# DJT777/xlstm-yolo-clean

Measured on NVIDIA B200. Metric: mLSTM chunkwise fwd+bwd TFLOP/s (algorithmic, 14*L*d*(L+d) per chunk), higher is better.
Workload: dtype bf16

## Files before the change

xlstm_yolo_clean_b200/csrc/tensor_kernels.cu:

```cuda
#include <atomic>
#include <mutex>
#include <set>
#include <type_traits>
#include <utility>

#include "common.cuh"
#include "sm100.cuh"

namespace mlstm {
namespace {

using namespace sm100;

constexpr int LT = 128;
constexpr int kWorkers = 256;
constexpr int kTcThreads = 320;
constexpr int kCtlWarp = 8, kScanWarp = 9;
constexpr int kNbAB = kWorkers + 32;
constexpr int kNbC = kWorkers + 64;
constexpr float kLog2e = 1.4426950408889634f;
enum { NB_A = 1, NB_B = 2, NB_C = 3, NB_PAIR0 = 4 };

struct GateBuf {
  static constexpr int oB = 0, oI = LT, oPm = 2 * LT, oY = 3 * LT, oF = 4 * LT, oMt = 5 * LT, oNt = 6 * LT,
// ... 1050 lines not shown
              v[4 * j4 + 0] *= cf.x * r_t;
              v[4 * j4 + 1] *= cf.y * r_t;
              v[4 * j4 + 2] *= cf.z * r_t;
              v[4 * j4 + 3] *= cf.w * r_t;
              rs += (v[4 * j4 + 0] + v[4 * j4 + 1]) + (v[4 * j4 + 2] + v[4 * j4 + 3]);
            }
          } else if (u == rb) {
            tmem_ld32(tS + lane_base + u * 32, v);
#pragma unroll
            for (int j4 = 0; j4 < 8; ++j4) {
              const float4 y = *reinterpret_cast<const float4*>(sy + u * 32 + 4 * j4);
              const float yy[4] = {y.x, y.y, y.z, y.w};
#pragma unroll
              for (int e = 0; e < 4; ++e) {
                const int j = 4 * j4 + e;
                float pv = v[j] * ex2_approx(x_t + yy[e]);
                pv = (REV ? j >= lane : j <= lane) ? pv : 0.f;
                rs += pv;
                v[j] = pv;
              }
            }
          } else {
#pragma unroll
            for (int j = 0; j < 32; ++j) v[j] = 0.f;
          }
          store_row32<T>(sP, row, u * 32, v);
        }
        srs[ch * LT + row] = rs;
      }
      fence_proxy_async_smem();
      tc_fence_before_sync();
      named_arrive(NB_B, kNbAB);
      {
        const float ab = __expf(g - b_t + i_t - m_next);
#pragma unroll 1
        for (int hf = 0; hf < 2; ++hf) {
          float kb[32];
#pragma unroll
          for (int j = 0; j < 4; ++j) {
            uint4 u = *reinterpret_cast<const uint4*>(sK + ch * SM::kTile + swz128(row, hf * 32 + 8 * j));
            float2 a0 = unpack2<T>(u.x), a1 = unpack2<T>(u.y), a2 = unpack2<T>(u.z), a3 = unpack2<T>(u.w);
            kb[8 * j + 0] = a0.x * ab; kb[8 * j + 1] = a0.y * ab; kb[8 * j + 2] = a1.x * ab; kb[8 * j + 3] = a1.y * ab;
            kb[8 * j + 4] = a2.x * ab; kb[8 * j + 5] = a2.y * ab; kb[8 * j + 6] = a3.x * ab; kb[8 * j + 7] = a3.y * ab;
          }
          store_row32<T>(sKb, row, ch * 64 + hf * 32, kb);
          const float cs = warp_colsum32(kb, lane);
          snp[rb * D + ch * 64 + hf * 32 + lane] = cs;
        }
        fence_proxy_async_smem();
        named_arrive(NB_A, kNbAB);
      }
      mbar_wait(&bar_h, par, 7);
      tc_fence_after_sync();
      {
        const float bq = __expf(b_t + m_run - m_t) * p.scale;
        const float den = bq * (sqn[row] + sqn[LT + row]) + srs[row] + srs[LT + row];
        const float nmax = fmaxf(fabsf(den), __expf(-m_t));
        const float inv = 1.f / (nmax + p.eps);
#pragma unroll 1
        for (int hf = 0; hf < 2; ++hf) {
          uint32_t hi[32], hx[32];
          tmem_ld32_nowait(tHi + lane_base + ch * 64 + hf * 32, hi);
          tmem_ld32_nowait(tHx + lane_base + ch * 64 + hf * 32, hx);
          tmem_ld_wait();
          float o[32];
#pragma unroll
          for (int j = 0; j < 32; ++j) o[j] = (__uint_as_float(hi[j]) + bq * __uint_as_float(hx[j])) * inv;
          store_row32<T>(sH, row, ch * 64 + hf * 32, o);
        }
        if (ch == 0 && row < n_valid) {
          p.n_out[(int64_t)bh * p.S + t0 + row] = nmax;
          p.m_out[(int64_t)bh * p.S + t0 + row] = m_t;
        }
        if (EPI) {
          uint8_t* sub = sH + ch * SM::kTile;
          const int64_t tok = (int64_t)(t0 + row);
          if (p.h_plain && row < n_valid) {
            uint4* dst = reinterpret_cast<uint4*>((T*)p.h_plain + b * p.h_sb + hh * p.h_sh + tok * p.h_ss + ch * 64);
#pragma unroll
            for (int j = 0; j < 8; ++j) dst[j] = *reinterpret_cast<const uint4*>(sub + swz128(row, 8 * j));
          }
          const void* xrow = p.x ? (const void*)((const uint16_t*)p.x + b * p.x_sb + hh * p.x_sh + tok * p.x_ss + ch * 64) : nullptr;
          ln_epilogue_slice<T, 128, 64>(sub, [](int r, int cc) { return swz128(r, cc & 63); }, row, ch * 64, ch, NB_PAIR0 + rb,
                                        fsm + SM::fStat, fsm + SM::fPar, xrow, p.xy_f16 != 0, p.ln_eps, row < n_valid);
        }
      }
      mbar_wait(&bar_dc, par, 6);
      tc_fence_after_sync();
      {
#pragma unroll
        for (int hf = 0; hf < 2; ++hf) {
          float v[32], t32[32];
          tmem_ld32(tDC + lane_base + ch * 64 + hf * 32, v);
#pragma unroll
          for (int j = 0; j < 32; ++j) {
            Creg[hf * 32 + j] = gbar * Creg[hf * 32 + j] + v[j];
            t32[j] = Creg[hf * 32 + j];
          }
          store_row32<T>(sC, row, ch * 64 + hf * 32, t32);
        }
        if (tid < D) {
          sNn[tid] = gbar * sNc[tid] + ((snp[tid] + snp[D + tid]) + (snp[2 * D + tid] + snp[3 * D + tid]));
          mbar_arrive(&bar_n);
        }
      }
      fence_proxy_async_smem();
      tc_fence_before_sync();
      named_arrive(NB_C, kNbC);
      m_run = m_next;
      cur ^= 1;
    }
    if (p.c_last) {
      float* dst = p.c_last + ((int64_t)bh * D + row) * D + ch * 64;
#pragma unroll
      for (int j = 0; j < 64; ++j) dst[j] = Creg[j];
      if (tid < D) p.n_last[(int64_t)bh * D + tid] = fsm[SM::fN + cur * D + tid];
      if (tid == 0) p.m_last[bh] = m_run;
    }
  }
  tc_fence_before_sync();
  __syncthreads();
  if (warp == kCtlWarp) tmem_dealloc<512>(tmem);
}

struct TcBwParams {
  int B, NH, S, NT;
  float eps, scale;
  const void *ig, *fg;
  int64_t ig_sb, ig_sh, ig_ss, fg_sb, fg_sh, fg_ss;
  const float* m0;
  const float *n_out, *m_out, *dc_last;
  void *di, *df;
  int64_t di_sb, di_sh, di_ss, df_sb, df_sh, df_ss;
  float* dc0;
  int rev;
  int sig;
  float cap;
  int acc_qk, acc_v, acc_g;
  int cs_rows, cs_off;
#ifdef MLSTM_TC_PROFILE
  long long* prof;
#endif
};

template <int D_>
struct BwSmem {
  static constexpr int D = D_;
  static constexpr int kTile = Lay<D>::kTile;
  static constexpr int kPTile = LT * 128;
  static constexpr int kState = Lay<D>::kState;
  static constexpr int kNST = D == 64 ? 1 : 2;
  static constexpr int kStage = 4 * kTile + kState;
  static constexpr int oQ = 0, oK = kTile, oV = 2 * kTile, odH = 3 * kTile, oCs = 4 * kTile;
  static constexpr int oQt = kNST * kStage;
  static constexpr int oSb = oQt + kTile;
  static constexpr int odS = oSb + 2 * kPTile;
  static constexpr int odQ = odS + 2 * kPTile;
  static constexpr int odV = odQ + kTile;
  static constexpr int odK = odV + kTile;
  static constexpr int odC = odK + kTile;
  static constexpr int oSmall = odC + kState;
  static constexpr int fGates = 0, fPart = 2 * GateBuf::kFloats, kSmallFloats = fPart + 12 * LT;
  static constexpr int kBytes = oSmall + kSmallFloats * 4 + 1024;
  static constexpr uint32_t kLoadBytes = 4 * kTile + kState;
  static constexpr bool kAlias = D == 64;
  static constexpr uint32_t cS = 0, cdSb = 128;
  static constexpr uint32_t cdV1 = D == 64 ? 0 : 256, cdV2 = cdV1 + D, cdK1 = D == 64 ? 128 : 320, cdK2 = cdK1 + D,
                            cdQa = D == 64 ? 256 : 384, cdQb = cdQa + D, cddC = D == 64 ? 384 : 448;
};

template <typename T, int D, bool REV, typename TO>
__global__ void __launch_bounds__(kTcThreads, 1)
tc_bw(const __grid_constant__ CUtensorMap mapQ, const __grid_constant__ CUtensorMap mapK,
          const __grid_constant__ CUtensorMap mapV, const __grid_constant__ CUtensorMap mapdH,
          const __grid_constant__ CUtensorMap mapCs, const __grid_constant__ CUtensorMap mapdQ,
          const __grid_constant__ CUtensorMap mapdK, const __grid_constant__ CUtensorMap mapdV, TcBwParams p) {
  constexpr bool kBf16 = std::is_same<T, __nv_bfloat16>::value;
  using SM = BwSmem<D>;
  using L = Lay<D>;
  constexpr int CW = L::CW;
  TC_PROF(200, 0);
  TC_PROF_CTA(0);
  extern __shared__ uint8_t smem_raw[];
  uint8_t* smem = smem_raw + ((1024u - (smem_u32(smem_raw) & 1023u)) & 1023u);
  uint8_t* sQ = smem + SM::oQ;
  uint8_t* sK = smem + SM::oK;
  uint8_t* sV = smem + SM::oV;
  uint8_t* sdH = smem + SM::odH;
  uint8_t* sQt = smem + SM::oQt;
  uint8_t* sSb = smem + SM::oSb;
  uint8_t* sdS = smem + SM::odS;
  uint8_t* sdQ = smem + SM::odQ;
  uint8_t* sdV = smem + SM::odV;
  uint8_t* sdK = smem + SM::odK;
  uint8_t* sCs = smem + SM::oCs;
  uint8_t* sdC = smem + SM::odC;
  float* fsm = (float*)(smem + SM::oSmall);
  __shared__ uint64_t bar_full[SM::kNST], bar_s, bar_q, bar_v, bar_k, bar_d, bar_b, bar_st, bar_g[2];
  __shared__ uint32_t tmem_base_s;

  const int tid = threadIdx.x, lane = tid & 31;
  const int warp = __shfl_sync(0xffffffffu, tid >> 5, 0);
  const int bh = blockIdx.x, b = bh / p.NH, hh = bh % p.NH;

  auto mt = [&](int c) { return REV ? p.NT - 1 - c : c; };
  auto load_stage = [&](int s, int c) {
    uint8_t* base = smem + s * SM::kStage;
    mbar_expect_tx(&bar_full[s], SM::kLoadBytes);
    tma_load_4d(base + SM::oQ, &mapQ, &bar_full[s], 0, mt(c) * LT, hh, b);
    tma_load_4d(base + SM::oK, &mapK, &bar_full[s], 0, mt(c) * LT, hh, b);
    tma_load_4d(base + SM::oV, &mapV, &bar_full[s], 0, mt(c) * LT, hh, b);
    tma_load_4d(base + SM::odH, &mapdH, &bar_full[s], 0, mt(c) * LT, hh, b);
    tma_load_4d(base + SM::oCs, &mapCs, &bar_full[s], 0, mt(c) * p.cs_rows + p.cs_off, hh, b);
  };
  if (tid == kCtlWarp * 32) {
    for (int s = 0; s < SM::kNST; ++s) mbar_init(&bar_full[s], 1);
    fence_mbar_init();
    grid_dep_wait();
    for (int s = 0; s < SM::kNST && s < p.NT; ++s) load_stage(s, p.NT - 1 - s);
  }
  if (tid == 0) {
    mbar_init(&bar_s, 1);
    mbar_init(&bar_b, 1);
    mbar_init(&bar_st, 1);
    mbar_init(&bar_q, 1);
    mbar_init(&bar_v, 1);
    mbar_init(&bar_k, 1);
    mbar_init(&bar_d, 1);
    mbar_init(&bar_g[0], 1);
    mbar_init(&bar_g[1], 1);
    fence_mbar_init();
  }
  if (warp == kCtlWarp) {
    tmem_alloc<512>(&tmem_base_s);
    if (lane == 0) {
      prefetch_tmap(&mapQ); prefetch_tmap(&mapK); prefetch_tmap(&mapV); prefetch_tmap(&mapdH);
      prefetch_tmap(&mapCs); prefetch_tmap(&mapdQ); prefetch_tmap(&mapdK); prefetch_tmap(&mapdV);
    }
  }
  grid_dep_wait();
  grid_dep_launch();
  const int rb = warp & 3, ch = (warp >> 2) & 1;
  const int row = rb * 32 + lane;
  const uint32_t lane_base = (uint32_t)(rb * 32) << 16;
  const int drow = rb * 16 + (lane & 15);
  const bool owns_c = warp < kCtlWarp && lane < 16 && rb * 16 < D;
  float dCreg[CW];
#pragma unroll
  for (int j = 0; j < CW; ++j) dCreg[j] = 0.f;
  if (warp < kCtlWarp) {
    if (p.dc_last && owns_c) {
      const float* src = p.dc_last + ((int64_t)bh * D + drow) * D + ch * CW;
#pragma unroll
      for (int j = 0; j < CW; ++j) dCreg[j] = src[j];
    }
    if (owns_c) store_cols<T, D>(sdC, drow, ch * CW, dCreg);
    fence_proxy_async_smem();
  }
  tc_fence_before_sync();
  __syncthreads();
  tc_fence_after_sync();
  const uint32_t tmem = tmem_base_s;
  const uint32_t tS = tmem + SM::cS, tdSb = tmem + SM::cdSb;
  const uint32_t tdV1 = tmem + SM::cdV1, tdV2 = tmem + SM::cdV2, tdK1 = tmem + SM::cdK1, tdK2 = tmem + SM::cdK2;
  const uint32_t tdQa = tmem + SM::cdQa, tdQb = tmem + SM::cdQb, tddC = tmem + SM::cddC;

  const T* ip = (const T*)p.ig + b * p.ig_sb + hh * p.ig_sh;
  const T* fp = (const T*)p.fg + b * p.fg_sb + hh * p.fg_sh;
  const float* mo = p.m_out + (int64_t)bh * p.S;
  const float* no = p.n_out + (int64_t)bh * p.S;
  if (warp == kCtlWarp) {
    constexpr uint32_t id_s = umma_idesc(128, 128, false, false, kBf16);
    constexpr uint32_t id_c = umma_idesc(64, D, true, true, kBf16);
    constexpr uint32_t id_k_mn = umma_idesc(128, D, false, true, kBf16);
    constexpr uint32_t id_mn_mn = umma_idesc(128, D, true, true, kBf16);
    constexpr uint32_t id_k_k = umma_idesc(128, D, false, false, kBf16);
    const uint64_t kQ0 = L::desc(smem_u32(sQ), 0), mQ0 = L::desc(smem_u32(sQ), SM::kTile);
    const uint64_t kK0 = L::desc(smem_u32(sK), 0), mK0 = L::desc(smem_u32(sK), SM::kTile);
    const uint64_t kV0 = L::desc(smem_u32(sV), 0);
    const uint64_t kH0 = L::desc(smem_u32(sdH), 0), mH0 = L::desc(smem_u32(sdH), SM::kTile);
    const uint64_t kCs0 = L::desc(smem_u32(sCs), 0);
    const uint64_t mQt = L::desc(smem_u32(sQt), D == 64 ? SM::kTile : 0);
    const uint64_t mSb = umma_smem_desc(smem_u32(sSb), SM::kPTile, 1024);
    const uint64_t kdS = umma_smem_desc(smem_u32(sdS), 0, 1024), mdS = umma_smem_desc(smem_u32(sdS), SM::kPTile, 1024);
    const uint64_t kdC = L::desc(smem_u32(sdC), 0), mdC = L::desc(smem_u32(sdC), SM::kState);
    auto issue_s = [&](int it) {
      const int s = it % SM::kNST;
      const uint32_t so = (uint32_t)s * SM::kStage;
      const uint64_t kQ = umma_desc_advance(kQ0, so), kK = umma_desc_advance(kK0, so);
      const uint64_t kH = umma_desc_advance(kH0, so), kV = umma_desc_advance(kV0, so);
      mbar_wait(&bar_full[s], (it / SM::kNST) & 1, 11);
      tc_fence_after_sync();
#pragma unroll
      for (int kk = 0; kk < D / 16; ++kk)
        umma_f16(tS, umma_desc_advance(kQ, kk * 32), umma_desc_advance(kK, kk * 32), id_s, kk > 0);
#pragma unroll
      for (int kk = 0; kk < D / 16; ++kk)
        umma_f16(tdSb, umma_desc_advance(kH, kk * 32), umma_desc_advance(kV, kk * 32), id_s, kk > 0);
      umma_commit(&bar_s);
    };

    if (elect_one()) issue_s(0);
    __syncwarp();

    for (int it = 0; it < p.NT; ++it) {
      const int c = p.NT - 1 - it, pb = it & 1;
      const uint32_t par = it & 1;
      const int t0 = mt(c) * LT, n_valid = min(LT, p.S - t0);
      const uint32_t so = (uint32_t)(it % SM::kNST) * SM::kStage;
      const uint64_t kQ = umma_desc_advance(kQ0, so), mQ = umma_desc_advance(mQ0, so);
      const uint64_t kK = umma_desc_advance(kK0, so), mK = umma_desc_advance(mK0, so);
      const uint64_t kV = umma_desc_advance(kV0, so), kCs = umma_desc_advance(kCs0, so);
      const uint64_t kH = umma_desc_advance(kH0, so), mH = umma_desc_advance(mH0, so);
      TC_PROF(it, 9);
      if (SM::kNST == 1 && c > 0 && lane == 0) {
        const int r = mt(c - 1) * LT;
        tma_prefetch_4d(&mapQ, 0, r, hh, b);
        tma_prefetch_4d(&mapK, 0, r, hh, b);
        tma_prefetch_4d(&mapV, 0, r, hh, b);
        tma_prefetch_4d(&mapdH, 0, r, hh, b);
        tma_prefetch_4d(&mapCs, 0, mt(c - 1) * p.cs_rows + p.cs_off, hh, b);
      }
      named_sync(NB_B, kNbAB);
      TC_PROF(it, 10);
      if (elect_one()) {
        tc_fence_after_sync();
#pragma unroll
        for (int kk = 0; kk < LT / 16; ++kk)
          umma_f16(tdK1, umma_desc_advance(mdS, kk * 2048), umma_desc_advance(mQ, kk * L::kAdvMN), id_mn_mn, kk > 0);
#pragma unroll
        for (int kk = 0; kk < D / 16; ++kk)
          umma_f16(tdK2, umma_desc_advance(kV, kk * 32), umma_desc_advance(kdC, kk * 32), id_k_k, kk > 0);
        umma_commit(&bar_k);
#pragma unroll
        for (int kk = 0; kk < LT / 16; ++kk)
          umma_f16(tdQa, umma_desc_advance(kdS, (kk / 4) * SM::kPTile + (kk % 4) * 32), umma_desc_advance(mK, kk * L::kAdvMN),
                   id_k_mn, kk > 0);
#pragma unroll
        for (int kk = 0; kk < D / 16; ++kk)
          umma_f16(tdQb, umma_desc_advance(kH, kk * 32), umma_desc_advance(kCs, kk * 32), id_k_k, kk > 0);
        umma_commit(&bar_q);
#pragma unroll
        for (int kk = 0; kk < D / 16; ++kk)
          umma_f16(tdV2, umma_desc_advance(kK, kk * 32), umma_desc_advance(mdC, kk * L::kAdvMN), id_k_mn, kk > 0);
        umma_commit(&bar_b);
      }
      __syncwarp();
      if (lane == 0) {
        tma_store_wait_read<0>();
        mbar_arrive(&bar_st);
      }
      __syncwarp();
      TC_PROF(it, 11);
      named_sync(NB_A, kNbAB);
      TC_PROF(it, 12);
      if (elect_one()) {
#pragma unroll
        for (int kk = 0; kk < LT / 16; ++kk)
          umma_f16(tddC, umma_desc_advance(mQt, kk * L::kAdvMN), umma_desc_advance(mH, kk * L::kAdvMN), id_c, kk > 0);
        umma_commit(&bar_d);
#pragma unroll
        for (int kk = 0; kk < LT / 16; ++kk)
          umma_f16(tdV1, umma_desc_advance(mSb, kk * 2048), umma_desc_advance(mH, kk * L::kAdvMN), id_mn_mn, kk > 0);
        umma_commit(&bar_v);
        if (!SM::kAlias && c > 0) issue_s(it + 1);
        if (SM::kNST == 1) {
          if (c > 0) {
            const int r = mt(c - 1) * LT;
            mbar_expect_tx(&bar_full[0], SM::kLoadBytes);
            mbar_wait(&bar_k, par, 21);
            tma_load_4d(sQ, &mapQ, &bar_full[0], 0, r, hh, b);
            tma_load_4d(sV, &mapV, &bar_full[0], 0, r, hh, b);
            mbar_wait(&bar_q, par, 24);
            tma_load_4d(sCs, &mapCs, &bar_full[0], 0, mt(c - 1) * p.cs_rows + p.cs_off, hh, b);
            mbar_wait(&bar_b, par, 22);
            tma_load_4d(sK, &mapK, &bar_full[0], 0, r, hh, b);
            mbar_wait(&bar_v, par, 25);
            tma_load_4d(sdH, &mapdH, &bar_full[0], 0, r, hh, b);
          }
        } else if (c >= SM::kNST) {
          mbar_wait(&bar_v, par, 25);
          load_stage(it % SM::kNST, c - SM::kNST);
        }
      }
      __syncwarp();
      TC_PROF(it, 13);
      named_sync(NB_C, kNbC);
      TC_PROF(it, 14);
      if (lane == 0) {
        if (p.acc_qk) {
          tma_reduce_add_4d(&mapdQ, sdQ, 0, t0, hh, b);
          tma_reduce_add_4d(&mapdK, sdK, 0, t0, hh, b);
        } else {
          tma_store_4d(&mapdQ, sdQ, 0, t0, hh, b);
          tma_store_4d(&mapdK, sdK, 0, t0, hh, b);
        }
        if (p.acc_v) tma_reduce_add_4d(&mapdV, sdV, 0, t0, hh, b);
        else tma_store_4d(&mapdV, sdV, 0, t0, hh, b);
        tma_store_commit();
      }
      __syncwarp();
      if (SM::kAlias && c > 0 && elect_one()) issue_s(it + 1);
      __syncwarp();
    }
    if (lane == 0) tma_store_wait_all<0>();
  } else if (warp == kScanWarp) {
    struct TileRaw {
      GateRaw<T> g;
      float4 mt, nt;
      float m_prev, m_next;
    };
    auto raw_of = [&](int c) {
      TileRaw r;
      const int t0 = mt(c) * LT, n_valid = min(LT, p.S - t0);
      r.g = load_gate_raw<T>(ip + (int64_t)t0 * p.ig_ss, p.ig_ss, fp + (int64_t)t0 * p.fg_ss, p.fg_ss, n_valid);
      if (lane * 4 < n_valid) {
        r.mt = *reinterpret_cast<const float4*>(mo + t0 + lane * 4);
        r.nt = *reinterpret_cast<const float4*>(no + t0 + lane * 4);
      } else {
        r.mt = make_float4(0.f, 0.f, 0.f, 0.f);
        r.nt = make_float4(1.f, 1.f, 1.f, 1.f);
      }
      if (!REV) {
        r.m_prev = c > 0 ? mo[t0 - 1] : (p.m0 ? p.m0[bh] : 0.f);
        r.m_next = mo[t0 + n_valid - 1];
      } else {
        r.m_prev = c > 0 ? mo[t0 + LT] : (p.m0 ? p.m0[bh] : 0.f);
        r.m_next = mo[t0];
      }
      return r;
    };
    auto publish = [&](float* gb, const TileRaw& r) {
      gate_scan_regs(gb, r.g, REV, p.sig != 0, p.cap);
      reinterpret_cast<float4*>(gb + GateBuf::oMt)[lane] = r.mt;
      reinterpret_cast<float4*>(gb + GateBuf::oNt)[lane] = r.nt;
      if (lane == 0) {
        gb[GateBuf::oScal + 2] = r.m_prev;
        gb[GateBuf::oScal + 3] = r.m_next;
      }
    };

    TileRaw raw = raw_of(p.NT - 1);
    float carry = 0.f;
    for (int n = 0; n < p.NT + 2; ++n) {
      if (n >= 2) {
      const int it = n - 2;
      const int c = p.NT - 1 - it, pb = it & 1;
      const int t0 = mt(c) * LT, n_valid = min(LT, p.S - t0);
      named_sync(NB_C, kNbC);
      {
        const float* sp = fsm + SM::fPart + pb * 6 * LT;
        const float* gb = fsm + SM::fGates + pb * GateBuf::kFloats;
        float acc[4], di[4];
#pragma unroll
        for (int e = 0; e < 4; ++e) {
          const int t = lane * 4 + e;
          acc[e] = (sp[0 * LT + t] + sp[1 * LT + t]) - (sp[2 * LT + t] + sp[3 * LT + t]);
          di[e] = sp[4 * LT + t] + sp[5 * LT + t];
        }
        float incl, own;
        if (!REV) {
          acc[2] += acc[3];
          acc[1] += acc[2];
          acc[0] += acc[1];
          incl = own = acc[0];
#pragma unroll
          for (int o = 1; o < 32; o <<= 1) {
            float u = __shfl_down_sync(0xffffffffu, incl, o);
            if (lane + o < 32) incl += u;
          }
        } else {
          acc[1] += acc[0];
          acc[2] += acc[1];
          acc[3] += acc[2];
          incl = own = acc[3];
#pragma unroll
          for (int o = 1; o < 32; o <<= 1) {
            float u = __shfl_up_sync(0xffffffffu, incl, o);
            if (lane >= o) incl += u;
          }
        }
        const float excl = incl - own + carry;
        TO* dip = (TO*)p.di + b * p.di_sb + hh * p.di_sh;
        TO* dfp = (TO*)p.df + b * p.df_sb + hh * p.df_sh;
#pragma unroll
        for (int e = 0; e < 4; ++e) {
          const int t = lane * 4 + e;
          if (t < n_valid) {
            const float dsig = p.sig ? 1.f - __expf(gb[GateBuf::oI + t]) : 1.f;
            float gi = di[e] * dsig * gb[GateBuf::oDi + t];
            float gf = (acc[e] + excl) * sigmoid_neg_f32(gb[GateBuf::oF + t]) * gb[GateBuf::oDf + t];
            TO* pi = dip + (int64_t)(t0 + t) * p.di_ss;
            TO* pf = dfp + (int64_t)(t0 + t) * p.df_ss;
            if (p.acc_g) {
              gi += to_f32<TO>(*pi);
              gf += to_f32<TO>(*pf);
            }
            *pi = from_f32<TO>(gi);
            *pf = from_f32<TO>(gf);
          }
        }
        carry += __shfl_sync(0xffffffffu, incl, REV ? 31 : 0);
      }
      __syncwarp();
      }
      if (n < p.NT) {
        publish(fsm + SM::fGates + (n & 1) * GateBuf::kFloats, raw);
        __syncwarp();
        if (lane == 0) mbar_arrive(&bar_g[n & 1]);
        if (n + 1 < p.NT) raw = raw_of(p.NT - 2 - n);
      }
    }
  } else {
    for (int it = 0; it < p.NT; ++it) {
      const int pb = it & 1;
      const uint32_t par = it & 1;
      const float* gb = fsm + SM::fGates + pb * GateBuf::kFloats;
      float* spart = fsm + SM::fPart + pb * 6 * LT;
      const int n_valid = min(LT, p.S - mt(p.NT - 1 - it) * LT);
      const bool valid = row < n_valid;
      const uint32_t so = (uint32_t)(it % SM::kNST) * SM::kStage;

      TC_PROF(it, 0);
      mbar_wait(&bar_g[pb], (it >> 1) & 1, 12);
      const float g = gb[GateBuf::oScal], m_prev = gb[GateBuf::oScal + 2], m_next = gb[GateBuf::oScal + 3];
      const float b_t = gb[GateBuf::oB + row], i_t = gb[GateBuf::oI + row];
      const float m_t = gb[GateBuf::oMt + row], n_t = gb[GateBuf::oNt + row];
      const float rinv = valid ? 1.f / (n_t + p.eps) : 0.f;
      const float bbar = valid ? __expf(b_t + m_prev - m_t) : 0.f;
      const float abar = __expf(g - b_t + i_t - m_next);
      const float gbar = __expf(g + m_prev - m_next);
      TC_PROF(it, 1);
      mbar_wait(&bar_full[it % SM::kNST], (it / SM::kNST) & 1, 13);
      uint32_t qs[CW / 2];
      {
        const float wq = p.scale * bbar * rinv;
#pragma unroll
        for (int j = 0; j < CW / 8; ++j) {
          const uint32_t off = L::swz(row, ch * CW + 8 * j);
          uint4 u = *reinterpret_cast<const uint4*>(sQ + so + off);
          qs[4 * j] = u.x; qs[4 * j + 1] = u.y; qs[4 * j + 2] = u.z; qs[4 * j + 3] = u.w;
          float2 a0 = unpack2<T>(u.x), a1 = unpack2<T>(u.y), a2 = unpack2<T>(u.z), a3 = unpack2<T>(u.w);
          u.x = pack2<T>(a0.x * wq, a0.y * wq);
          u.y = pack2<T>(a1.x * wq, a1.y * wq);
          u.z = pack2<T>(a2.x * wq, a2.y * wq);
          u.w = pack2<T>(a3.x * wq, a3.y * wq);
          *reinterpret_cast<uint4*>(sQt + off) = u;
        }
      }
      mbar_wait(&bar_s, par, 14);
      tc_fence_after_sync();
      TC_PROF(it, 2);
      {
        const float x_t = valid ? (b_t - m_t) * kLog2e + log2f(rinv) : -INFINITY;
        const float* sy = gb + GateBuf::oY;
        const float* scf = gb + GateBuf::oCf;
#pragma unroll 1
        for (int u = ch; u < 4; u += 2) {
          float v[32], w[32];
          if (REV ? u >= rb : u <= rb) {
            uint32_t rv[32], rw[32];
            tmem_ld32_nowait(tS + lane_base + u * 32, rv);
            tmem_ld32_nowait(tdSb + lane_base + u * 32, rw);
            tmem_ld_wait();
            if (u != rb) {
              const float r_t = ex2_approx(x_t + gb[GateBuf::oScal + 4 + u]);
#pragma unroll
              for (int j4 = 0; j4 < 8; ++j4) {
                const float4 cf = *reinterpret_cast<const float4*>(scf + u * 32 + 4 * j4);
                const float cc[4] = {cf.x, cf.y, cf.z, cf.w};
#pragma unroll
                for (int e = 0; e < 4; ++e) {
                  const int j = 4 * j4 + e;
                  const float wg = cc[e] * r_t;
                  v[j] = __uint_as_float(rv[j]) * wg;
                  w[j] = __uint_as_float(rw[j]) * wg;
                }
              }
            } else {
#pragma unroll
              for (int j4 = 0; j4 < 8; ++j4) {
                const float4 y = *reinterpret_cast<const float4*>(sy + u * 32 + 4 * j4);
                const float yy[4] = {y.x, y.y, y.z, y.w};
#pragma unroll
                for (int e = 0; e < 4; ++e) {
                  const int j = 4 * j4 + e;
                  float wg = ex2_approx(x_t + yy[e]);
                  wg = (REV ? j >= lane : j <= lane) ? wg : 0.f;
                  v[j] = __uint_as_float(rv[j]) * wg;
                  w[j] = __uint_as_float(rw[j]) * wg;
                }
              }
            }
          } else {
            if (it > 0) continue;
#pragma unroll
            for (int j = 0; j < 32; ++j) { v[j] = 0.f; w[j] = 0.f; }
          }
          store_row32<T>(sSb, row, u * 32, v);
          store_row32<T>(sdS, row, u * 32, w);
        }
      }
      fence_proxy_async_smem();
      tc_fence_before_sync();
      named_arrive(NB_B, kNbAB);
      TC_PROF(it, 3);
      uint32_t ks[CW / 2], vs[CW / 2];
#pragma unroll
      for (int j = 0; j < CW / 8; ++j) {
        const uint32_t off = L::swz(row, ch * CW + 8 * j);
        uint4 uk = *reinterpret_cast<const uint4*>(sK + so + off);
        ks[4 * j] = uk.x; ks[4 * j + 1] = uk.y; ks[4 * j + 2] = uk.z; ks[4 * j + 3] = uk.w;
        uint4 uv = *reinterpret_cast<const uint4*>(sV + so + off);
        vs[4 * j] = uv.x; vs[4 * j + 1] = uv.y; vs[4 * j + 2] = uv.z; vs[4 * j + 3] = uv.w;
      }
      fence_proxy_async_smem();
      named_arrive(NB_A, kNbAB);
      TC_PROF(it, 4);
      {
        uint32_t ra[CW], rq[CW];
        float o[CW];
        float dot;
        mbar_wait(&bar_k, par, 18);
        tc_fence_after_sync();
        TC_PROF(it, 5);
        tmem_ld_nowait(tdK1 + lane_base + ch * CW, ra);
        tmem_ld_nowait(tdK2 + lane_base + ch * CW, rq);
        tmem_ld_wait();
        dot = 0.f;
#pragma unroll
        for (int j = 0; j < CW / 2; ++j) {
          o[2 * j] = p.scale * __uint_as_float(ra[2 * j]) + abar * __uint_as_float(rq[2 * j]);
          o[2 * j + 1] = p.scale * __uint_as_float(ra[2 * j + 1]) + abar * __uint_as_float(rq[2 * j + 1]);
          float2 kv = unpack2<T>(ks[j]);
          dot += kv.x * o[2 * j] + kv.y * o[2 * j + 1];
        }
        mbar_wait(&bar_st, par, 19);
        store_cols<TO, D>(sdK, row, ch * CW, o);
        spart[(1 * 2 + ch) * LT + row] = dot;
        mbar_wait(&bar_q, par, 16);
        tc_fence_after_sync();
        TC_PROF(it, 6);
        tmem_ld_nowait(tdQa + lane_base + ch * CW, ra);
        tmem_ld_nowait(tdQb + lane_base + ch * CW, rq);
        tmem_ld_wait();
        const float wb = bbar * rinv;
        dot = 0.f;
#pragma unroll
        for (int j = 0; j < CW / 2; ++j) {
          o[2 * j] = p.scale * (__uint_as_float(ra[2 * j]) + wb * __uint_as_float(rq[2 * j]));
          o[2 * j + 1] = p.scale * (__uint_as_float(ra[2 * j + 1]) + wb * __uint_as_float(rq[2 * j + 1]));
          float2 qv = unpack2<T>(qs[j]);
          dot += qv.x * o[2 * j] + qv.y * o[2 * j + 1];
        }
        store_cols<TO, D>(sdQ, row, ch * CW, o);
        spart[(0 * 2 + ch) * LT + row] = dot;
      }
      mbar_wait(&bar_d, par, 15);
      tc_fence_after_sync();
      TC_PROF(it, 7);
      {
        float v[CW];
        tmem_ld(tddC + lane_base + ch * CW, v);
        if (owns_c) {
#pragma unroll
          for (int j = 0; j < CW; ++j) dCreg[j] = gbar * dCreg[j] + v[j];
          store_cols<T, D>(sdC, drow, ch * CW, dCreg);
        }
      }
      {
        uint32_t ra[CW], rq[CW];
        float o[CW];
        float dot;
        mbar_wait(&bar_v, par, 17);
        tc_fence_after_sync();
        tmem_ld_nowait(tdV1 + lane_base + ch * CW, ra);
        tmem_ld_nowait(tdV2 + lane_base + ch * CW, rq);
        tmem_ld_wait();
        dot = 0.f;
#pragma unroll
        for (int j = 0; j < CW / 2; ++j) {
          o[2 * j] = p.scale * __uint_as_float(ra[2 * j]) + abar * __uint_as_float(rq[2 * j]);
          o[2 * j + 1] = p.scale * __uint_as_float(ra[2 * j + 1]) + abar * __uint_as_float(rq[2 * j + 1]);
          float2 vv = unpack2<T>(vs[j]);
          dot += vv.x * o[2 * j] + vv.y * o[2 * j + 1];
        }
        store_cols<TO, D>(sdV, row, ch * CW, o);
        spart[(2 * 2 + ch) * LT + row] = dot;
      }
      fence_proxy_async_smem();
      tc_fence_before_sync();
      named_arrive(NB_C, kNbC);
      TC_PROF(it, 8);
    }
    if (p.dc0 && owns_c) {
      float* dst = p.dc0 + ((int64_t)bh * D + drow) * D + ch * CW;
#pragma unroll
      for (int j = 0; j < CW; ++j) dst[j] = dCreg[j];
    }
  }
  TC_PROF(200, 1);
  tc_fence_before_sync();
  __syncthreads();
  TC_PROF(200, 2);
  TC_PROF_CTA(1);
  if (warp == kCtlWarp) tmem_dealloc<512>(tmem);
}

#ifdef MLSTM_TC_PROFILE
std::atomic<long long*> g_prof{nullptr};
#define TC_SET_PROF(p, off) (p).prof = g_prof.load() ? g_prof.load() + (off) : nullptr
#else
#define TC_SET_PROF(p, off)
#endif

int num_sms() {
  static int n = 0;
  if (!n) {
    int dev = 0;
    cudaGetDevice(&dev);
    cudaDeviceGetAttribute(&n, cudaDevAttrMultiProcessorCount, dev);
  }
  return n;
}

template <typename K>
cudaError_t ensure_smem(K kern, int bytes) {
  static std::mutex mu;
  static std::set<std::pair<const void*, int>> done;
  int dev = 0;
  cudaGetDevice(&dev);
  const std::pair<const void*, int> key(reinterpret_cast<const void*>(kern), dev);
  {
    std::lock_guard<std::mutex> g(mu);
    if (done.count(key)) return cudaSuccess;
  }
  cudaError_t e = cudaFuncSetAttribute(kern, cudaFuncAttributeMaxDynamicSharedMemorySize, bytes);
  if (e == cudaSuccess) {
    std::lock_guard<std::mutex> g(mu);
    done.insert(key);
  }
  return e;
}

int pdl_mode() {
  static int v = -1;
  if (v < 0) {
    const char* e = getenv("MLSTM_B200_PDL");
    v = e ? (e[0] - '0') : 2;
    if (v < 0 || v > 2) v = 2;
  }
  return v;
}
template <typename... KArgs, typename... Args>
cudaError_t launch_pdl(bool use_pdl, void (*kern)(KArgs...), int grid, int block, size_t smem, cudaStream_t st, Args&&... args) {
  cudaLaunchConfig_t cfg = {};
  cfg.gridDim = dim3(grid), cfg.blockDim = dim3(block), cfg.dynamicSmemBytes = smem, cfg.stream = st;
  cudaLaunchAttribute attr[1];
  attr[0].id = cudaLaunchAttributeProgrammaticStreamSerialization;
  attr[0].val.programmaticStreamSerializationAllowed = 1;
  cfg.attrs = attr, cfg.numAttrs = use_pdl ? 1 : 0;
  return cudaLaunchKernelEx(&cfg, kern, std::forward<Args>(args)...);
}

template <typename T, int D>
int launch_fw(const TcFwParams& p, const CUtensorMap& mq, const CUtensorMap& mk, const CUtensorMap& mv,
              const CUtensorMap& mh, const CUtensorMap& mcs, cudaStream_t st) {
  using SM = FwSmem<D>;
  auto kern = p.epi ? (p.rev ? tc_fw<T, D, true, true> : tc_fw<T, D, false, true>)
                    : (p.rev ? tc_fw<T, D, true, false> : tc_fw<T, D, false, false>);
  MLSTM_CUDA_CHECK(ensure_smem(kern, SM::kBytes));
  MLSTM_CUDA_CHECK(launch_pdl(pdl_mode() != 0, kern, p.B * p.NH, kTcThreads, SM::kBytes, st, mq, mk, mv, mh, mcs, p));
  count_launch();
  MLSTM_CUDA_CHECK(cudaGetLastError());
  return 0;
}

template <typename... KArgs, typename... Args>
cudaError_t launch_pair_pdl(bool use_pdl, void (*kern)(KArgs...), int grid, int block, size_t smem, cudaStream_t st,
                            Args&&... args) {
  cudaLaunchConfig_t cfg = {};
  cfg.gridDim = dim3(grid), cfg.blockDim = dim3(block), cfg.dynamicSmemBytes = smem, cfg.stream = st;
  cudaLaunchAttribute attr[2];
  attr[0].id = cudaLaunchAttributeClusterDimension;
  attr[0].val.clusterDim.x = 2, attr[0].val.clusterDim.y = 1, attr[0].val.clusterDim.z = 1;
  attr[1].id = cudaLaunchAttributeProgrammaticStreamSerialization;
  attr[1].val.programmaticStreamSerializationAllowed = 1;
  cfg.attrs = attr, cfg.numAttrs = use_pdl ? 2 : 1;
  return cudaLaunchKernelEx(&cfg, kern, std::forward<Args>(args)...);
}

template <typename T, int D>
auto fw_rect_kernel(bool epi, bool rev) {
  return epi ? (rev ? tc_fw_rect<T, D, true, true> : tc_fw_rect<T, D, false, true>)
             : (rev ? tc_fw_rect<T, D, true, false> : tc_fw_rect<T, D, false, false>);
}

template <typename T, int D>
int launch_fw_rect(const TcFwParams& p, const CUtensorMap& mq, const CUtensorMap& mk, const CUtensorMap& mv,
                   const CUtensorMap& mh, const CUtensorMap& mcs, cudaStream_t st) {
  using SM = FwSmem<D>;
  auto kern = fw_rect_kernel<T, D>(p.epi != 0, p.rev != 0);
  if (p.epi) {
    MLSTM_CUDA_CHECK(ensure_smem(kern, SM::kBytesPair));
    MLSTM_CUDA_CHECK(launch_pair_pdl(pdl_mode() != 0, kern, 2 * p.B * p.NH, kTcThreads, SM::kBytesPair, st, mq, mk, mv, mh, mcs, p));
  } else {
    MLSTM_CUDA_CHECK(ensure_smem(kern, SM::kBytes));
    MLSTM_CUDA_CHECK(launch_pdl(pdl_mode() != 0, kern, 2 * p.B * p.NH, kTcThreads, SM::kBytes, st, mq, mk, mv, mh, mcs, p));
  }
  count_launch();
  MLSTM_CUDA_CHECK(cudaGetLastError());
  return 0;
}

template <typename T>
int launch_fw_d128(const TcFwParams& p, const CUtensorMap& mq, const CUtensorMap& mk, const CUtensorMap& mv,
                   const CUtensorMap& mh, const CUtensorMap& mcs, cudaStream_t st) {
  auto kern = p.epi ? (p.rev ? tc_fw_d128<T, true, true> : tc_fw_d128<T, false, true>)
                    : (p.rev ? tc_fw_d128<T, true, false> : tc_fw_d128<T, false, false>);
  MLSTM_CUDA_CHECK(ensure_smem(kern, FwSmem128::kBytes));
  kern<<<p.B * p.NH, kTcThreads, FwSmem128::kBytes, st>>>(mq, mk, mv, mh, mcs, p);
  count_launch();
  MLSTM_CUDA_CHECK(cudaGetLastError());
  return 0;
}

template <typename T, int D, typename TO = T>
int launch_bw(const TcBwParams& p, const CUtensorMap& mq, const CUtensorMap& mk, const CUtensorMap& mv,
              const CUtensorMap& mdh, const CUtensorMap& mcs, const CUtensorMap& mdq, const CUtensorMap& mdk,
              const CUtensorMap& mdv, cudaStream_t st) {
  using SM = BwSmem<D>;
  auto kern = p.rev ? tc_bw<T, D, true, TO> : tc_bw<T, D, false, TO>;
  MLSTM_CUDA_CHECK(ensure_smem(kern, SM::kBytes));
  MLSTM_CUDA_CHECK(launch_pdl(pdl_mode() == 1, kern, p.B * p.NH, kTcThreads, SM::kBytes, st, mq, mk, mv, mdh, mcs, mdq, mdk, mdv, p));
  MLSTM_CUDA_CHECK(cudaGetLastError());
  return 0;
}

bool tma_ok(const mlstm_b200_tensor& t) {
  return ((uintptr_t)t.ptr & 15) == 0 && t.stride[3] == 1 && (t.stride[0] % 8) == 0 && (t.stride[1] % 8) == 0 &&
         (t.stride[2] % 8) == 0;
}
// ... 366 lines not shown
```

Before: 251.1.

## Fold gate scales into operands and accumulate dK/dQ partials in single TMEM tiles

The backward tensor-core kernel now pre-scales dH (instead of Q) and V by their gate factors in shared memory. This lets the two dK matmuls and the two dQ matmuls accumulate into one TMEM region each, instead of two regions combined later in registers. The dC state-gradient GEMM is issued in the first batch, the Cs state tile gets its own barrier so most MMAs can start before it arrives, and the MMA/TMA issue order and barrier set are reorganized. The aim is to remove epilogue FMAs and TMEM loads and to overlap the loads better. In exchange there are extra shared-memory rewrites of V, possible bf16 rounding of the pre-scaled operands, and more intricate synchronization.

```diff
diff --git a/xlstm_yolo_clean_b200/csrc/tensor_kernels.cu b/xlstm_yolo_clean_b200/csrc/tensor_kernels.cu
--- a/xlstm_yolo_clean_b200/csrc/tensor_kernels.cu
+++ b/xlstm_yolo_clean_b200/csrc/tensor_kernels.cu
@@ -1226,8 +1226,8 @@
   static constexpr int kNST = D == 64 ? 1 : 2;
   static constexpr int kStage = 4 * kTile + kState;
   static constexpr int oQ = 0, oK = kTile, oV = 2 * kTile, odH = 3 * kTile, oCs = 4 * kTile;
-  static constexpr int oQt = kNST * kStage;
-  static constexpr int oSb = oQt + kTile;
+  static constexpr int odHt = kNST * kStage;
+  static constexpr int oSb = odHt + kTile;
   static constexpr int odS = oSb + 2 * kPTile;
   static constexpr int odQ = odS + 2 * kPTile;
   static constexpr int odV = odQ + kTile;
@@ -1236,11 +1236,10 @@
   static constexpr int oSmall = odC + kState;
   static constexpr int fGates = 0, fPart = 2 * GateBuf::kFloats, kSmallFloats = fPart + 12 * LT;
   static constexpr int kBytes = oSmall + kSmallFloats * 4 + 1024;
-  static constexpr uint32_t kLoadBytes = 4 * kTile + kState;
-  static constexpr bool kAlias = D == 64;
-  static constexpr uint32_t cS = 0, cdSb = 128;
-  static constexpr uint32_t cdV1 = D == 64 ? 0 : 256, cdV2 = cdV1 + D, cdK1 = D == 64 ? 128 : 320, cdK2 = cdK1 + D,
-                            cdQa = D == 64 ? 256 : 384, cdQb = cdQa + D, cddC = D == 64 ? 384 : 448;
+  static constexpr uint32_t kLoadBytes = 4 * kTile;
+  static constexpr uint32_t cS = 0, cdSb = 128, cddC = cdSb;
+  static constexpr uint32_t cdQ = 256, cdK = cdQ + D, cdV1 = cdK + D, cdV2 = cdV1 + D;
+  static_assert(cdV2 + D <= 512, "TMEM columns");
 };
 
 template <typename T, int D, bool REV, typename TO>
@@ -1261,7 +1260,7 @@
   uint8_t* sK = smem + SM::oK;
   uint8_t* sV = smem + SM::oV;
   uint8_t* sdH = smem + SM::odH;
-  uint8_t* sQt = smem + SM::oQt;
+  uint8_t* sdHt = smem + SM::odHt;
   uint8_t* sSb = smem + SM::oSb;
   uint8_t* sdS = smem + SM::odS;
   uint8_t* sdQ = smem + SM::odQ;
@@ -1270,7 +1269,7 @@
   uint8_t* sCs = smem + SM::oCs;
   uint8_t* sdC = smem + SM::odC;
   float* fsm = (float*)(smem + SM::oSmall);
-  __shared__ uint64_t bar_full[SM::kNST], bar_s, bar_q, bar_v, bar_k, bar_d, bar_b, bar_st, bar_g[2];
+  __shared__ uint64_t bar_full[SM::kNST], bar_cs[SM::kNST], bar_s, bar_q, bar_v, bar_k, bar_st, bar_g[2];
   __shared__ uint32_t tmem_base_s;
 
   const int tid = threadIdx.x, lane = tid & 31;
@@ -1285,22 +1284,24 @@
     tma_load_4d(base + SM::oK, &mapK, &bar_full[s], 0, mt(c) * LT, hh, b);
     tma_load_4d(base + SM::oV, &mapV, &bar_full[s], 0, mt(c) * LT, hh, b);
     tma_load_4d(base + SM::odH, &mapdH, &bar_full[s], 0, mt(c) * LT, hh, b);
-    tma_load_4d(base + SM::oCs, &mapCs, &bar_full[s], 0, mt(c) * p.cs_rows + p.cs_off, hh, b);
+    mbar_expect_tx(&bar_cs[s], SM::kState);
+    tma_load_4d(base + SM::oCs, &mapCs, &bar_cs[s], 0, mt(c) * p.cs_rows + p.cs_off, hh, b);
   };
   if (tid == kCtlWarp * 32) {
-    for (int s = 0; s < SM::kNST; ++s) mbar_init(&bar_full[s], 1);
+    for (int s = 0; s < SM::kNST; ++s) {
+      mbar_init(&bar_full[s], 1);
+      mbar_init(&bar_cs[s], 1);
+    }
     fence_mbar_init();
     grid_dep_wait();
     for (int s = 0; s < SM::kNST && s < p.NT; ++s) load_stage(s, p.NT - 1 - s);
   }
   if (tid == 0) {
     mbar_init(&bar_s, 1);
-    mbar_init(&bar_b, 1);
     mbar_init(&bar_st, 1);
     mbar_init(&bar_q, 1);
     mbar_init(&bar_v, 1);
     mbar_init(&bar_k, 1);
-    mbar_init(&bar_d, 1);
     mbar_init(&bar_g[0], 1);
     mbar_init(&bar_g[1], 1);
     fence_mbar_init();
@@ -1336,8 +1337,8 @@
   tc_fence_after_sync();
   const uint32_t tmem = tmem_base_s;
   const uint32_t tS = tmem + SM::cS, tdSb = tmem + SM::cdSb;
-  const uint32_t tdV1 = tmem + SM::cdV1, tdV2 = tmem + SM::cdV2, tdK1 = tmem + SM::cdK1, tdK2 = tmem + SM::cdK2;
-  const uint32_t tdQa = tmem + SM::cdQa, tdQb = tmem + SM::cdQb, tddC = tmem + SM::cddC;
+  const uint32_t tdQ = tmem + SM::cdQ, tdK = tmem + SM::cdK, tdV1 = tmem + SM::cdV1, tdV2 = tmem + SM::cdV2;
+  const uint32_t tddC = tmem + SM::cddC;
 
   const T* ip = (const T*)p.ig + b * p.ig_sb + hh * p.ig_sh;
   const T* fp = (const T*)p.fg + b * p.fg_sb + hh * p.fg_sh;
@@ -1349,12 +1350,12 @@
     constexpr uint32_t id_k_mn = umma_idesc(128, D, false, true, kBf16);
     constexpr uint32_t id_mn_mn = umma_idesc(128, D, true, true, kBf16);
     constexpr uint32_t id_k_k = umma_idesc(128, D, false, false, kBf16);
-    const uint64_t kQ0 = L::desc(smem_u32(sQ), 0), mQ0 = L::desc(smem_u32(sQ), SM::kTile);
+    const uint64_t kQ0 = L::desc(smem_u32(sQ), 0), mQ0 = L::desc(smem_u32(sQ), D == 64 ? SM::kTile : 0);
     const uint64_t kK0 = L::desc(smem_u32(sK), 0), mK0 = L::desc(smem_u32(sK), SM::kTile);
     const uint64_t kV0 = L::desc(smem_u32(sV), 0);
     const uint64_t kH0 = L::desc(smem_u32(sdH), 0), mH0 = L::desc(smem_u32(sdH), SM::kTile);
     const uint64_t kCs0 = L::desc(smem_u32(sCs), 0);
-    const uint64_t mQt = L::desc(smem_u32(sQt), D == 64 ? SM::kTile : 0);
+    const uint64_t kHt = L::desc(smem_u32(sdHt), 0), mHt = L::desc(smem_u32(sdHt), SM::kTile);
     const uint64_t mSb = umma_smem_desc(smem_u32(sSb), SM::kPTile, 1024);
     const uint64_t kdS = umma_smem_desc(smem_u32(sdS), 0, 1024), mdS = umma_smem_desc(smem_u32(sdS), SM::kPTile, 1024);
     const uint64_t kdC = L::desc(smem_u32(sdC), 0), mdC = L::desc(smem_u32(sdC), SM::kState);
@@ -1385,7 +1386,7 @@
       const uint64_t kQ = umma_desc_advance(kQ0, so), mQ = umma_desc_advance(mQ0, so);
       const uint64_t kK = umma_desc_advance(kK0, so), mK = umma_desc_advance(mK0, so);
       const uint64_t kV = umma_desc_advance(kV0, so), kCs = umma_desc_advance(kCs0, so);
-      const uint64_t kH = umma_desc_advance(kH0, so), mH = umma_desc_advance(mH0, so);
+      const uint64_t mH = umma_desc_advance(mH0, so);
       TC_PROF(it, 9);
       if (SM::kNST == 1 && c > 0 && lane == 0) {
         const int r = mt(c - 1) * LT;
@@ -1401,23 +1402,31 @@
         tc_fence_after_sync();
 #pragma unroll
         for (int kk = 0; kk < LT / 16; ++kk)
-          umma_f16(tdK1, umma_desc_advance(mdS, kk * 2048), umma_desc_advance(mQ, kk * L::kAdvMN), id_mn_mn, kk > 0);
-#pragma unroll
-        for (int kk = 0; kk < D / 16; ++kk)
-          umma_f16(tdK2, umma_desc_advance(kV, kk * 32), umma_desc_advance(kdC, kk * 32), id_k_k, kk > 0);
-        umma_commit(&bar_k);
-#pragma unroll
-        for (int kk = 0; kk < LT / 16; ++kk)
-          umma_f16(tdQa, umma_desc_advance(kdS, (kk / 4) * SM::kPTile + (kk % 4) * 32), umma_desc_advance(mK, kk * L::kAdvMN),
-                   id_k_mn, kk > 0);
-#pragma unroll
-        for (int kk = 0; kk < D / 16; ++kk)
-          umma_f16(tdQb, umma_desc_advance(kH, kk * 32), umma_desc_advance(kCs, kk * 32), id_k_k, kk > 0);
-        umma_commit(&bar_q);
+          umma_f16(tdV1, umma_desc_advance(mSb, kk * 2048), umma_desc_advance(mH, kk * L::kAdvMN), id_mn_mn, kk > 0);
 #pragma unroll
         for (int kk = 0; kk < D / 16; ++kk)
           umma_f16(tdV2, umma_desc_advance(kK, kk * 32), umma_desc_advance(mdC, kk * L::kAdvMN), id_k_mn, kk > 0);
-        umma_commit(&bar_b);
+        umma_commit(&bar_v);
+#pragma unroll
+        for (int kk = 0; kk < LT / 16; ++kk)
+          umma_f16(tdK, umma_desc_advance(mdS, kk * 2048), umma_desc_advance(mQ, kk * L::kAdvMN), id_mn_mn, kk > 0);
+#pragma unroll
+        for (int kk = 0; kk < D / 16; ++kk)
+          umma_f16(tdK, umma_desc_advance(kV, kk * 32), umma_desc_advance(kdC, kk * 32), id_k_k, true);
+#pragma unroll
+        for (int kk = 0; kk < LT / 16; ++kk)
+          umma_f16(tddC, umma_desc_advance(mQ, kk * L::kAdvMN), umma_desc_advance(mHt, kk * L::kAdvMN), id_c, kk > 0);
+#pragma unroll
+        for (int kk = 0; kk < LT / 16; ++kk)
+          umma_f16(tdQ, umma_desc_advance(kdS, (kk / 4) * SM::kPTile + (kk % 4) * 32), umma_desc_advance(mK, kk * L::kAdvMN),
+                   id_k_mn, kk > 0);
+        umma_commit(&bar_k);
+        mbar_wait(&bar_cs[it % SM::kNST], (it / SM::kNST) & 1, 26);
+        tc_fence_after_sync();
+#pragma unroll
+        for (int kk = 0; kk < D / 16; ++kk)
+          umma_f16(tdQ, umma_desc_advance(kHt, kk * 32), umma_desc_advance(kCs, kk * 32), id_k_k, true);
+        umma_commit(&bar_q);
       }
       __syncwarp();
       if (lane == 0) {
@@ -1426,34 +1435,26 @@
       }
       __syncwarp();
       TC_PROF(it, 11);
+      if (SM::kNST == 1 && c > 0 && elect_one()) {
+        const int r = mt(c - 1) * LT;
+        mbar_expect_tx(&bar_full[0], SM::kLoadBytes);
+        mbar_wait(&bar_v, par, 25);
+        tma_load_4d(sdH, &mapdH, &bar_full[0], 0, r, hh, b);
+        mbar_wait(&bar_k, par, 21);
+        tma_load_4d(sQ, &mapQ, &bar_full[0], 0, r, hh, b);
+        tma_load_4d(sV, &mapV, &bar_full[0], 0, r, hh, b);
+        tma_load_4d(sK, &mapK, &bar_full[0], 0, r, hh, b);
+        mbar_wait(&bar_q, par, 24);
+        mbar_expect_tx(&bar_cs[0], SM::kState);
+        tma_load_4d(sCs, &mapCs, &bar_cs[0], 0, mt(c - 1) * p.cs_rows + p.cs_off, hh, b);
+      }
+      __syncwarp();
+      TC_PROF(it, 12);
       named_sync(NB_A, kNbAB);
-      TC_PROF(it, 12);
       if (elect_one()) {
-#pragma unroll
-        for (int kk = 0; kk < LT / 16; ++kk)
-          umma_f16(tddC, umma_desc_advance(mQt, kk * L::kAdvMN), umma_desc_advance(mH, kk * L::kAdvMN), id_c, kk > 0);
-        umma_commit(&bar_d);
-#pragma unroll
-        for (int kk = 0; kk < LT / 16; ++kk)
-          umma_f16(tdV1, umma_desc_advance(mSb, kk * 2048), umma_desc_advance(mH, kk * L::kAdvMN), id_mn_mn, kk > 0);
-        umma_commit(&bar_v);
-        if (!SM::kAlias && c > 0) issue_s(it + 1);
-        if (SM::kNST == 1) {
-          if (c > 0) {
-            const int r = mt(c - 1) * LT;
-            mbar_expect_tx(&bar_full[0], SM::kLoadBytes);
-            mbar_wait(&bar_k, par, 21);
-            tma_load_4d(sQ, &mapQ, &bar_full[0], 0, r, hh, b);
-            tma_load_4d(sV, &mapV, &bar_full[0], 0, r, hh, b);
-            mbar_wait(&bar_q, par, 24);
-            tma_load_4d(sCs, &mapCs, &bar_full[0], 0, mt(c - 1) * p.cs_rows + p.cs_off, hh, b);
-            mbar_wait(&bar_b, par, 22);
-            tma_load_4d(sK, &mapK, &bar_full[0], 0, r, hh, b);
-            mbar_wait(&bar_v, par, 25);
-            tma_load_4d(sdH, &mapdH, &bar_full[0], 0, r, hh, b);
-          }
-        } else if (c >= SM::kNST) {
-          mbar_wait(&bar_v, par, 25);
+        if (c > 0) issue_s(it + 1);
+        if (SM::kNST > 1 && c >= SM::kNST) {
+          mbar_wait(&bar_q, par, 24);
           load_stage(it % SM::kNST, c - SM::kNST);
         }
       }
@@ -1473,8 +1474,6 @@
         else tma_store_4d(&mapdV, sdV, 0, t0, hh, b);
         tma_store_commit();
       }
-      __syncwarp();
-      if (SM::kAlias && c > 0 && elect_one()) issue_s(it + 1);
       __syncwarp();
     }
     if (lane == 0) tma_store_wait_all<0>();
@@ -1606,27 +1605,41 @@
       const float gbar = __expf(g + m_prev - m_next);
       TC_PROF(it, 1);
       mbar_wait(&bar_full[it % SM::kNST], (it / SM::kNST) & 1, 13);
-      uint32_t qs[CW / 2];
+      uint32_t qs[CW / 2], ks[CW / 2], vs[CW / 2];
       {
-        const float wq = p.scale * bbar * rinv;
+        const float wh = p.scale * bbar * rinv;
 #pragma unroll
         for (int j = 0; j < CW / 8; ++j) {
           const uint32_t off = L::swz(row, ch * CW + 8 * j);
-          uint4 u = *reinterpret_cast<const uint4*>(sQ + so + off);
-          qs[4 * j] = u.x; qs[4 * j + 1] = u.y; qs[4 * j + 2] = u.z; qs[4 * j + 3] = u.w;
+          const uint4 uq = *reinterpret_cast<const uint4*>(sQ + so + off);
+          qs[4 * j] = uq.x; qs[4 * j + 1] = uq.y; qs[4 * j + 2] = uq.z; qs[4 * j + 3] = uq.w;
+          const uint4 uv = *reinterpret_cast<const uint4*>(sV + so + off);
+          vs[4 * j] = uv.x; vs[4 * j + 1] = uv.y; vs[4 * j + 2] = uv.z; vs[4 * j + 3] = uv.w;
+          uint4 u = *reinterpret_cast<const uint4*>(sdH + so + off);
           float2 a0 = unpack2<T>(u.x), a1 = unpack2<T>(u.y), a2 = unpack2<T>(u.z), a3 = unpack2<T>(u.w);
-          u.x = pack2<T>(a0.x * wq, a0.y * wq);
-          u.y = pack2<T>(a1.x * wq, a1.y * wq);
-          u.z = pack2<T>(a2.x * wq, a2.y * wq);
-          u.w = pack2<T>(a3.x * wq, a3.y * wq);
-          *reinterpret_cast<uint4*>(sQt + off) = u;
+          u.x = pack2<T>(a0.x * wh, a0.y * wh);
+          u.y = pack2<T>(a1.x * wh, a1.y * wh);
+          u.z = pack2<T>(a2.x * wh, a2.y * wh);
+          u.w = pack2<T>(a3.x * wh, a3.y * wh);
+          *reinterpret_cast<uint4*>(sdHt + off) = u;
         }
       }
       mbar_wait(&bar_s, par, 14);
       tc_fence_after_sync();
       TC_PROF(it, 2);
+#pragma unroll
+      for (int j = 0; j < CW / 8; ++j) {
+        uint4 u;
+        float2 a0 = unpack2<T>(vs[4 * j]), a1 = unpack2<T>(vs[4 * j + 1]), a2 = unpack2<T>(vs[4 * j + 2]),
+               a3 = unpack2<T>(vs[4 * j + 3]);
+        u.x = pack2<T>(a0.x * abar, a0.y * abar);
+        u.y = pack2<T>(a1.x * abar, a1.y * abar);
+        u.z = pack2<T>(a2.x * abar, a2.y * abar);
+        u.w = pack2<T>(a3.x * abar, a3.y * abar);
+        *reinterpret_cast<uint4*>(sV + so + L::swz(row, ch * CW + 8 * j)) = u;
+      }
       {
-        const float x_t = valid ? (b_t - m_t) * kLog2e + log2f(rinv) : -INFINITY;
+        const float x_t = valid ? (b_t - m_t) * kLog2e + log2f(p.scale * rinv) : -INFINITY;
         const float* sy = gb + GateBuf::oY;
         const float* scf = gb + GateBuf::oCf;
 #pragma unroll 1
@@ -1675,93 +1688,80 @@
           store_row32<T>(sdS, row, u * 32, w);
         }
       }
+#pragma unroll
+      for (int j = 0; j < CW / 8; ++j) {
+        const uint4 uk = *reinterpret_cast<const uint4*>(sK + so + L::swz(row, ch * CW + 8 * j));
+        ks[4 * j] = uk.x; ks[4 * j + 1] = uk.y; ks[4 * j + 2] = uk.z; ks[4 * j + 3] = uk.w;
+      }
       fence_proxy_async_smem();
       tc_fence_before_sync();
       named_arrive(NB_B, kNbAB);
       TC_PROF(it, 3);
-      uint32_t ks[CW / 2], vs[CW / 2];
-#pragma unroll
-      for (int j = 0; j < CW / 8; ++j) {
-        const uint32_t off = L::swz(row, ch * CW + 8 * j);
-        uint4 uk = *reinterpret_cast<const uint4*>(sK + so + off);
-        ks[4 * j] = uk.x; ks[4 * j + 1] = uk.y; ks[4 * j + 2] = uk.z; ks[4 * j + 3] = uk.w;
-        uint4 uv = *reinterpret_cast<const uint4*>(sV + so + off);
-        vs[4 * j] = uv.x; vs[4 * j + 1] = uv.y; vs[4 * j + 2] = uv.z; vs[4 * j + 3] = uv.w;
-      }
-      fence_proxy_async_smem();
-      named_arrive(NB_A, kNbAB);
-      TC_PROF(it, 4);
+      uint32_t ra[CW];
+      float o[CW];
+      float dot;
       {
-        uint32_t ra[CW], rq[CW];
-        float o[CW];
-        float dot;
-        mbar_wait(&bar_k, par, 18);
-        tc_fence_after_sync();
-        TC_PROF(it, 5);
-        tmem_ld_nowait(tdK1 + lane_base + ch * CW, ra);
-        tmem_ld_nowait(tdK2 + lane_base + ch * CW, rq);
-        tmem_ld_wait();
-        dot = 0.f;
-#pragma unroll
-        for (int j = 0; j < CW / 2; ++j) {
-          o[2 * j] = p.scale * __uint_as_float(ra[2 * j]) + abar * __uint_as_float(rq[2 * j]);
-          o[2 * j + 1] = p.scale * __uint_as_float(ra[2 * j + 1]) + abar * __uint_as_float(rq[2 * j + 1]);
-          float2 kv = unpack2<T>(ks[j]);
-          dot += kv.x * o[2 * j] + kv.y * o[2 * j + 1];
-        }
-        mbar_wait(&bar_st, par, 19);
-        store_cols<TO, D>(sdK, row, ch * CW, o);
-        spart[(1 * 2 + ch) * LT + row] = dot;
-        mbar_wait(&bar_q, par, 16);
-        tc_fence_after_sync();
-        TC_PROF(it, 6);
-        tmem_ld_nowait(tdQa + lane_base + ch * CW, ra);
-        tmem_ld_nowait(tdQb + lane_base + ch * CW, rq);
-        tmem_ld_wait();
-        const float wb = bbar * rinv;
-        dot = 0.f;
-#pragma unroll
-        for (int j = 0; j < CW / 2; ++j) {
-          o[2 * j] = p.scale * (__uint_as_float(ra[2 * j]) + wb * __uint_as_float(rq[2 * j]));
-          o[2 * j + 1] = p.scale * (__uint_as_float(ra[2 * j + 1]) + wb * __uint_as_float(rq[2 * j + 1]));
-          float2 qv = unpack2<T>(qs[j]);
-          dot += qv.x * o[2 * j] + qv.y * o[2 * j + 1];
-        }
-        store_cols<TO, D>(sdQ, row, ch * CW, o);
-        spart[(0 * 2 + ch) * LT + row] = dot;
-      }
-      mbar_wait(&bar_d, par, 15);
-      tc_fence_after_sync();
-      TC_PROF(it, 7);
-      {
-        float v[CW];
-        tmem_ld(tddC + lane_base + ch * CW, v);
-        if (owns_c) {
-#pragma unroll
-          for (int j = 0; j < CW; ++j) dCreg[j] = gbar * dCreg[j] + v[j];
-          store_cols<T, D>(sdC, drow, ch * CW, dCreg);
-        }
-      }
-      {
-        uint32_t ra[CW], rq[CW];
-        float o[CW];
-        float dot;
+        uint32_t rq[CW];
         mbar_wait(&bar_v, par, 17);
         tc_fence_after_sync();
+        TC_PROF(it, 4);
         tmem_ld_nowait(tdV1 + lane_base + ch * CW, ra);
         tmem_ld_nowait(tdV2 + lane_base + ch * CW, rq);
         tmem_ld_wait();
         dot = 0.f;
 #pragma unroll
         for (int j = 0; j < CW / 2; ++j) {
-          o[2 * j] = p.scale * __uint_as_float(ra[2 * j]) + abar * __uint_as_float(rq[2 * j]);
-          o[2 * j + 1] = p.scale * __uint_as_float(ra[2 * j + 1]) + abar * __uint_as_float(rq[2 * j + 1]);
+          o[2 * j] = __uint_as_float(ra[2 * j]) + abar * __uint_as_float(rq[2 * j]);
+          o[2 * j + 1] = __uint_as_float(ra[2 * j + 1]) + abar * __uint_as_float(rq[2 * j + 1]);
           float2 vv = unpack2<T>(vs[j]);
           dot += vv.x * o[2 * j] + vv.y * o[2 * j + 1];
         }
+        mbar_wait(&bar_st, par, 19);
         store_cols<TO, D>(sdV, row, ch * CW, o);
         spart[(2 * 2 + ch) * LT + row] = dot;
       }
+      mbar_wait(&bar_k, par, 18);
+      tc_fence_after_sync();
+      TC_PROF(it, 5);
+      {
+        float v[CW];
+        tmem_ld(tddC + lane_base + ch * CW, v);
+        tc_fence_before_sync();
+        named_arrive(NB_A, kNbAB);
+        if (owns_c) {
+#pragma unroll
+          for (int j = 0; j < CW; ++j) dCreg[j] = gbar * dCreg[j] + v[j];
+          store_cols<T, D>(sdC, drow, ch * CW, dCreg);
+        }
+      }
+      tmem_ld_nowait(tdK + lane_base + ch * CW, ra);
+      tmem_ld_wait();
+      dot = 0.f;
+#pragma unroll
+      for (int j = 0; j < CW / 2; ++j) {
+        o[2 * j] = __uint_as_float(ra[2 * j]);
+        o[2 * j + 1] = __uint_as_float(ra[2 * j + 1]);
+        float2 kv = unpack2<T>(ks[j]);
+        dot += kv.x * o[2 * j] + kv.y * o[2 * j + 1];
+      }
+      store_cols<TO, D>(sdK, row, ch * CW, o);
+      spart[(1 * 2 + ch) * LT + row] = dot;
+      mbar_wait(&bar_q, par, 16);
+      tc_fence_after_sync();
+      TC_PROF(it, 6);
+      tmem_ld_nowait(tdQ + lane_base + ch * CW, ra);
+      tmem_ld_wait();
+      dot = 0.f;
+#pragma unroll
+      for (int j = 0; j < CW / 2; ++j) {
+        o[2 * j] = __uint_as_float(ra[2 * j]);
+        o[2 * j + 1] = __uint_as_float(ra[2 * j + 1]);
+        float2 qv = unpack2<T>(qs[j]);
+        dot += qv.x * o[2 * j] + qv.y * o[2 * j + 1];
+      }
+      store_cols<TO, D>(sdQ, row, ch * CW, o);
+      spart[(0 * 2 + ch) * LT + row] = dot;
+      TC_PROF(it, 7);
       fence_proxy_async_smem();
       tc_fence_before_sync();
       named_arrive(NB_C, kNbC);
```

New measurement: 250.7, median of 6. No clear change (-0.2%).
